# Meng-333/SRADSGAN

Hardware: AMD Instinct MI355X
Metric: training images/sec (216x216, x4) (higher is better)
Workload: dtype f32 (split-bf16 products: 3 bf16 MFMA terms per fp32 multiply, fp32 accumulate)

## Files before the change

### sradsgan_amd/csrc/conv_fast_fprop.hip

```cpp
#include "conv_dev.h"

namespace srhip {

int g_fast_ablate = 0;


template <int BM, int BN, int WM, int WN, int BK, int MATH = 0>
__global__ __launch_bounds__(WM* WN * 64) void fast_conv_kernel(const float* __restrict__ src,
                                                                 const float* __restrict__ wt,
                                                                 const float* __restrict__ bias,
                                                                 const float* __restrict__ residual,
                                                                 const float* __restrict__ rowscale,
                                                                 const float* __restrict__ chanscale,
                                                                 const float* __restrict__ actmask,
                                                                 float* __restrict__ dst, FastGeom g, int nblk_m,
                                                                 int nblk_n) {
  constexpr int NT = WM * WN * 64;
  constexpr int WTM = BM / WM, WTN = BN / WN;
  constexpr int TM = WTM / 32, TN = WTN / 32;
  constexpr int LS = BK + 4;
  constexpr int QPR = BK / 4;
  constexpr int RPP = NT / QPR;
  constexpr int AR = (BM + RPP - 1) / RPP, BR = (BN + RPP - 1) / RPP;
  constexpr int STAGE = (BM + BN) * LS;
// ... 910 lines not shown
    const int orow = pt >> 16, ocol = pt & 0xffff;
    const int arow = orow < pg.PH ? orow * pg.PWP + ocol : 0;
#pragma unroll
    for (int sidx = 0; sidx < 9; ++sidx) {
      const int T = 2 * sidx + wk;
      const int par = T >= 9 ? 1 : 0, tap = T - 9 * par;
      const int th = tap / 3, tw = tap - 3 * th;
      const int a_th = (g.dh0 + th * g.dhs) - pg.lo_h, a_tw = (g.dw0 + tw * g.dws) - pg.lo_w;
      const int pr = arow + a_th * pg.PWP + a_tw;
      aoffS[sidx][t] = par * PATCH_B + pr * 64 + (((2 * khalf) ^ ((pr >> 2) & 3)) << 4);
    }
  }
  int boffk[TN];
#pragma unroll
  for (int u = 0; u < TN; ++u) {
    const int row = u * 32 + l31;
    boffk[u] = 2 * PATCH_B + wk * BSTAGE_B + row * 64 + (((2 * khalf) ^ ((row >> 2) & 3)) << 4);
  }
  f32x16 acc[TM][TN];
#pragma unroll
  for (int t = 0; t < TM; ++t)
#pragma unroll
    for (int u = 0; u < TN; ++u)
#pragma unroll
      for (int r = 0; r < 16; ++r) acc[t][u][r] = 0.f;

  auto do_step = [&](auto sc, auto lastc, int cc0) {
    constexpr int S = decltype(sc)::value;
    constexpr bool LAST = decltype(lastc)::value != 0;
    constexpr int NEWER = S == 0 ? 2 : S == 1 ? 4 : S == 2 ? 3 : (S >= 3 && S <= 5) ? 2 : S == 6 ? (LAST ? 2 : 4) : S == 7 ? (LAST ? 2 : 3) : (LAST ? 0 : 2);
    wait_vmcnt<NEWER>();
    asm volatile("s_waitcnt lgkmcnt(0)" ::: "memory");
    __builtin_amdgcn_s_barrier();
    asm volatile("" ::: "memory");
    if (S == 0) {
      issue_a(1, 0, cc0 + 1);
      issue_a(1, 1, cc0 + 1);
    }
    if (S == 1) issue_a(1, 2, cc0 + 1);
    if (!LAST && S == 5) {
      issue_a(0, 0, cc0 + 2);
      issue_a(0, 1, cc0 + 2);
    }
    if (!LAST && S == 6) issue_a(0, 2, cc0 + 2);
#pragma unroll
    for (int d = 0; d < 2; ++d) {
      constexpr int T0 = 2 * S + 4;
      const int T = T0 + d;
      if (T < 18) issue_b(T % NST, T % 9, cc0 + T / 9);
      else if (!LAST) issue_b(T % NST, (T - 18) % 9, cc0 + 2 + (T - 18) / 9);
    }
    if (S == 2) {
      convert_piece(1, 0);
      convert_piece(1, 1);
    }
    if (S == 3) convert_piece(1, 2);
    if (!LAST && S == 7) {
      convert_piece(0, 0);
      convert_piece(0, 1);
    }
    if (!LAST && S == 8) convert_piece(0, 2);
    const char* sb = lds + ((2 * S) % NST) * BSTAGE_B;
    bf16x8_t ah[TM], al[TM], bh[TN], bl[TN];
#pragma unroll
    for (int t = 0; t < TM; ++t) {
      ah[t] = *reinterpret_cast<const bf16x8_t*>(lds + aoffS[S][t]);
      al[t] = *reinterpret_cast<const bf16x8_t*>(lds + (aoffS[S][t] ^ 16));
    }
#pragma unroll
    for (int u = 0; u < TN; ++u) {
      bh[u] = *reinterpret_cast<const bf16x8_t*>(sb + boffk[u]);
      bl[u] = *reinterpret_cast<const bf16x8_t*>(sb + (boffk[u] ^ 16));
    }
#pragma unroll
    for (int i = 0; i < 3 * TM * TN; ++i) {
      const int grp = i / (TM * TN), t = (i % (TM * TN)) / TN, u = i % TN;
      acc[t][u] = mma16<0>(grp == 0 ? al[t] : ah[t], grp == 1 ? bl[u] : bh[u], acc[t][u]);
    }
  };
  auto do_pair = [&](auto lastc, int cc0) {
    do_step(IC<0>(), lastc, cc0);
    do_step(IC<1>(), lastc, cc0);
    do_step(IC<2>(), lastc, cc0);
    do_step(IC<3>(), lastc, cc0);
    do_step(IC<4>(), lastc, cc0);
    do_step(IC<5>(), lastc, cc0);
    do_step(IC<6>(), lastc, cc0);
    do_step(IC<7>(), lastc, cc0);
    do_step(IC<8>(), lastc, cc0);
  };

  wait_vmcnt<4>();
#pragma unroll
  for (int k = 0; k < MAXP; ++k) convert_piece(0, k);
  for (int cc0 = 0; cc0 + 2 < CC; cc0 += 2) do_pair(IC<0>(), cc0);
  do_pair(IC<1>(), CC - 2);

  __syncthreads();
  {
    float* xl = reinterpret_cast<float*>(lds);
#pragma unroll
    for (int t = 0; t < TM; ++t)
#pragma unroll
      for (int r = 0; r < 16; ++r) xl[((wave * TM + t) * 16 + r) * 64 + lane] = wk ? acc[t][0][r] : acc[t][1][r];
    __syncthreads();
    const int pw = wave ^ 1;
#pragma unroll
    for (int t = 0; t < TM; ++t)
#pragma unroll
      for (int r = 0; r < 16; ++r) {
        const float o = xl[((pw * TM + t) * 16 + r) * 64 + lane];
        acc[t][0][r] = (wk ? acc[t][1][r] : acc[t][0][r]) + o;
      }
    __syncthreads();
  }

  const int flags = EPI >= 0 ? EPI : g.flags;
  constexpr int WTN = 32;
  float* wl = reinterpret_cast<float*>(lds) + wave * (32 * WTN);
  constexpr int QPRW = WTN / 4;
  constexpr int NRD = 32 * QPRW / 64;
#pragma unroll
  for (int t = 0; t < TM; ++t) {
#pragma unroll
    for (int r = 0; r < 16; ++r) wl[((r & 3) + 8 * (r >> 2) + 4 * khalf) * WTN + l31] = acc[t][0][r];
    asm volatile("s_waitcnt lgkmcnt(0)" ::: "memory");
    float4 vq[NRD];
    EpiOps eo[NRD];
    unsigned dpx[NRD];
    int nq[NRD];
    bool okq[NRD];
#pragma unroll
    for (int j = 0; j < NRD; ++j) {
      const int idx = j * 64 + lane;
      const int row = idx / QPRW, cq = idx - row * QPRW;
      vq[j] = *reinterpret_cast<const float4*>(wl + row * WTN + cq * 4);
      const int r = wm * 64 + t * 32 + row;
      const int pt = pix_tab[r];
      const int orow = pt >> 16, ocol = pt & 0xffff;
      const int oh = oh0 + orow, ow = ow0 + ocol;
      const int n = n0 + wk * WTN + cq * 4;
      okq[j] = !(orow >= pg.PH || oh >= g.OH || ow >= g.OW || n >= g.K);
      dpx[j] = okq[j] ? (unsigned)((img * g.Hd + oh) * g.Wd + ow) : 0u;
      nq[j] = okq[j] ? n : 0;
      eo[j] = epi_fetch(dpx[j], nq[j], flags, g, bias, residual, nullptr, actmask, dst, false);
    }
#pragma unroll
    for (int j = 0; j < NRD; ++j)
      if (okq[j]) epi_finish(vq[j], eo[j], dpx[j], nq[j], flags, g, dst, false);
    if (t + 1 < TM) asm volatile("s_waitcnt lgkmcnt(0)" ::: "memory");
  }
}

template <int ND, bool MASK>
__global__ __launch_bounds__(256) void narrow_conv_kernel(const float* __restrict__ src, const float* __restrict__ wt,
                                                           const float* __restrict__ bias, float* __restrict__ dst,
                                                           FastGeom g, int tiles_h, int tiles_w, int lo_h, int lo_w,
                                                           const unsigned long long* __restrict__ smask) {
  constexpr int PW = 16, PH = 16, PWP = PW + 2, PR = (PH + 2) * PWP;
  __shared__ __attribute__((aligned(16))) float4 lds[2][PR * 4];
  const int tid = threadIdx.x;
  const int tpi = tiles_h * tiles_w;
  const int img = blockIdx.x / tpi;
  const int prem = blockIdx.x - img * tpi;
  const int ty = prem / tiles_w, tx = prem - ty * tiles_w;
  const int oh0 = ty * PH, ow0 = tx * PW;
  const int py = tid >> 4, px = tid & 15;

  int soff[6];
  int sdst[6];
  unsigned long long mw[MASK ? 6 : 1];
#pragma unroll
  for (int i = 0; i < 6; ++i) {
    const int e = tid + i * 256;
    soff[i] = -1;
    sdst[i] = 0;
    if (MASK) mw[i] = 0ull;
    if (e < PR * 4) {
      const int row = e >> 2, q = e & 3;
      const int pi = row / PWP, pj = row - pi * PWP;
      const int sh = oh0 + lo_h + pi, sw = ow0 + lo_w + pj;
      sdst[i] = row * 4 + (q ^ (row & 3));
      if (sh >= 0 && sh < g.Hs && sw >= 0 && sw < g.Ws) {
        soff[i] = ((img * g.Hs + sh) * g.Ws + sw) * g.lds + q * 4;
        if (MASK) mw[i] = smask[(img * g.Hs + sh) * g.Ws + sw];
      } else {
        soff[i] = -2;
      }
    }
  }
  const int CC = g.C / 16;
  float4 stage[6];
  auto fetch = [&](int cc) {
#pragma unroll
    for (int i = 0; i < 6; ++i) {
      stage[i] = soff[i] >= 0 ? *reinterpret_cast<const float4*>(src + (size_t)soff[i] + cc * 16) : make_float4(0.f, 0.f, 0.f, 0.f);
      if (MASK) {
        const unsigned b = (unsigned)(mw[i] >> (cc * 16 + (tid & 3) * 4));
        stage[i].x = (b & 1u) ? stage[i].x : stage[i].x * g.slope;
        stage[i].y = (b & 2u) ? stage[i].y : stage[i].y * g.slope;
        stage[i].z = (b & 4u) ? stage[i].z : stage[i].z * g.slope;
        stage[i].w = (b & 8u) ? stage[i].w : stage[i].w * g.slope;
      }
    }
  };
  auto commit = [&](int buf) {
#pragma unroll
    for (int i = 0; i < 6; ++i)
      if (soff[i] != -1) lds[buf][sdst[i]] = stage[i];
  };
  float acc[ND];
#pragma unroll
  for (int n = 0; n < ND; ++n) acc[n] = 0.f;

  fetch(0);
  commit(0);
  __syncthreads();
  for (int cc = 0; cc < CC; ++cc) {
    const int buf = cc & 1;
    if (cc + 1 < CC) fetch(cc + 1);
#pragma unroll 1
    for (int tap = 0; tap < 9; ++tap) {
      {
        const int th = tap / 3, tw = tap - th * 3;
        const int a_th = (g.dh0 + th * g.dhs) - lo_h, a_tw = (g.dw0 + tw * g.dws) - lo_w;
        const int row = (py + a_th) * PWP + px + a_tw;
        const int wk = ((g.kh0 + th * g.khs) * g.KW + (g.kw0 + tw * g.kws)) * g.C + cc * 16;
#pragma unroll
        for (int q = 0; q < 4; ++q) {
          const float4 v = lds[buf][row * 4 + (q ^ (row & 3))];
#pragma unroll
          for (int n = 0; n < ND; ++n) {
            const float* w = wt + (size_t)n * g.ldw + wk + q * 4;
            acc[n] = fmaf(v.x, w[0], acc[n]);
            acc[n] = fmaf(v.y, w[1], acc[n]);
            acc[n] = fmaf(v.z, w[2], acc[n]);
            acc[n] = fmaf(v.w, w[3], acc[n]);
          }
        }
      }
    }
    if (cc + 1 < CC) commit(buf ^ 1);
    __syncthreads();
  }
  const int oh = oh0 + py, ow = ow0 + px;
  if (oh < g.OH && ow < g.OW) {
    const size_t dpix = ((size_t)img * g.Hd + oh) * g.Wd + ow;
#pragma unroll
    for (int n = 0; n < ND; ++n) {
      if (n < g.K) {
        float v = acc[n];
        if (g.flags & SRHIP_EPI_BIAS) v += bias[n];
        if (g.flags & SRHIP_EPI_LRELU) v = v > 0.f ? v : v * g.slope;
        dst[dpix * g.ldd + n] = v;
      }
    }
  }
}

__global__ __launch_bounds__(256) void dot_conv_kernel(const float* __restrict__ src, const float* __restrict__ wt,
                                                        const float* __restrict__ bias, float* __restrict__ dst, FastGeom g) {
  const int lane = threadIdx.x & 63;
  const int m = blockIdx.x * 4 + (threadIdx.x >> 6);
  if (m >= g.M) return;
  const int ow = m % g.OW, t = m / g.OW;
  const int oh = t % g.OH, n = t / g.OH;
  float acc = 0.f;
  for (int th = 0; th < g.TH; ++th) {
    const int sh = oh * g.ss + g.dh0 + th * g.dhs;
    if (sh < 0 || sh >= g.Hs) continue;
    for (int tw = 0; tw < g.TW; ++tw) {
      const int sw = ow * g.ss + g.dw0 + tw * g.dws;
      if (sw < 0 || sw >= g.Ws) continue;
      const float* xp = src + ((size_t)(n * g.Hs + sh) * g.Ws + sw) * g.lds;
      const float* wp = wt + (size_t)((g.kh0 + th * g.khs) * g.KW + (g.kw0 + tw * g.kws)) * g.C;
      for (int c = lane * 4; c < g.C; c += 256) {
        const float4 a = *reinterpret_cast<const float4*>(xp + c);
        const float4 b = *reinterpret_cast<const float4*>(wp + c);
        acc = fmaf(a.x, b.x, acc);
        acc = fmaf(a.y, b.y, acc);
        acc = fmaf(a.z, b.z, acc);
        acc = fmaf(a.w, b.w, acc);
      }
    }
  }
#pragma unroll
  for (int o = 32; o >= 1; o >>= 1) acc += __shfl_xor(acc, o, 64);
  if (lane == 0) {
    float v = acc;
    if (g.flags & SRHIP_EPI_BIAS) v += bias[0];
    if (g.flags & SRHIP_EPI_LRELU) v = v > 0.f ? v : v * g.slope;
    dst[((size_t)(n * g.Hd + oh * g.dsd + g.ph) * g.Wd + ow * g.dsd + g.pw) * g.ldd] = v;
  }
}

__global__ void fast_pack_kernel(const float* __restrict__ w, float* __restrict__ packed, int cout, int cin, int kh,
                                 int kw, int mode) {
  const int idx = blockIdx.x * blockDim.x + threadIdx.x;
  const int total = cout * cin * kh * kw;
  if (idx >= total) return;
  const int khkw = kh * kw;
  if (mode == 0) {
    const int co = idx / (khkw * cin);
    const int rem = idx - co * khkw * cin;
    const int tap = rem / cin, ci = rem - tap * cin;
    fast_pack_store(packed, total, idx, w[((size_t)co * cin + ci) * khkw + tap], cout, cin, khkw);
  } else {
    const int ci = idx / (khkw * cout);
    const int rem = idx - ci * khkw * cout;
    const int tap = rem / cout, co = rem - tap * cout;
    fast_pack_store(packed, total, idx, w[((size_t)co * cin + ci) * khkw + tap], cin, cout, khkw);
  }
}

static bool shape_ok(int csrc, int kh, int kw) { return csrc % 16 == 0 && kh * kw <= 32 && kh == kw; }
bool fast_fwd_ok(int cin, int cout, int kh, int kw) { return shape_ok(cin, kh, kw); }
bool fast_dgrad_ok(int cin, int cout, int kh, int kw) { return shape_ok(cout, kh, kw); }
bool fast_wgrad_ok(int cin, int cout, int kh, int kw) { return cin % 16 == 0 && cout % 4 == 0 && kh == kw; }

int fast_pack_weight(const float* w, float* packed, int cout, int cin, int kh, int kw, int mode, hipStream_t st) {
  const long total = (long)cout * cin * kh * kw;
  hipLaunchKernelGGL(fast_pack_kernel, dim3(cdiv(total, 256)), dim3(256), 0, st, w, packed, cout, cin, kh, kw, mode);
  return check_launch("fast_pack_weight");
}

thread_local Dst2Request g_dst2_req;
thread_local ResRequest g_res_req;
thread_local PhaseRequest g_phase_req;
thread_local SrcMaskRequest g_src_mask_req;
int g_conv_math = 0;
int g_patch_ks = 1;
int g_fast_cfg = 0;
int g_phase_batch = 1;

static bool plan_patch(const FastGeom& g, PatchGeom* pg, double min_eff = 0.70) {
  if (g.TH != 3 || g.TW != 3 || g.ss != 1 || g.dsd != 1 || g.ph != 0 || g.pw != 0) return false;
  if ((g.dhs != 1 && g.dhs != -1) || (g.dws != 1 && g.dws != -1)) return false;
  if (g.Hd != g.OH || g.Wd != g.OW) return false;
  double best = 0.0;
  for (int pw = 4; pw <= 64 && pw <= g.OW + 3; ++pw) {
    int ph = 128 / pw;
    if (ph > g.OH) ph = g.OH;
    if (ph < 1 || (ph + 2) * (pw + 2) > 192) continue;
    const long tiles = (long)cdiv(g.OH, ph) * cdiv(g.OW, pw);
    const double eff = (double)g.OH * g.OW / ((double)tiles * 128.0) + 1e-6 * (double)(pw - pw % 16) / pw;
    if (eff > best + 1e-9) {
      best = eff;
      pg->PH = ph; pg->PW = pw;
    }
  }
  if (best < min_eff || best <= 0.0) return false;
  pg->tiles_h = cdiv(g.OH, pg->PH);
  pg->tiles_w = cdiv(g.OW, pg->PW);
  pg->PWP = pg->PW + 2;
  pg->PR = (pg->PH + 2) * pg->PWP;
  pg->npieces = cdiv(pg->PR, 16);
  pg->lo_h = g.dhs > 0 ? g.dh0 : g.dh0 + 2 * g.dhs;
  pg->lo_w = g.dws > 0 ? g.dw0 : g.dw0 + 2 * g.dws;
  const int a = pg->PW >> 4;
  const int nfull = pg->PH * a < 8 ? pg->PH * a : 8;
  auto base = [&](int q) { return ((q / a) * pg->PWP + (q % a) * 16) & 15; };
  int fin[8], nf = 0, singles[8], ns = 0;
  bool used[8] = {false, false, false, false, false, false, false, false};
  for (int q = 0; q < nfull; ++q) {
    if (used[q]) continue;
    used[q] = true;
    int partner = -1;
    for (int p2 = q + 1; p2 < nfull; ++p2)
      if (!used[p2] && base(p2) == base(q)) {
        partner = p2;
        break;
      }
    if (partner >= 0) {
      used[partner] = true;
      fin[nf++] = q;
      fin[nf++] = partner;
    } else {
      singles[ns++] = q;
    }
  }
  for (int i = 0; i < ns; ++i) fin[nf++] = singles[i];
  for (int q = nfull; q < 8; ++q) fin[nf++] = q;
  pg->gmap = 0;
  for (int i = 0; i < 8; ++i) pg->gmap |= (unsigned)(fin[i] & 15) << (4 * i);
  return true;
}

long pp_sign_tiles(int n, int h, int w, int cout) {
  if (cout < 128 || cout % 128 != 0) return 0;
  FastGeom g;
// ... 409 lines not shown
```

### sradsgan_amd/csrc/conv_igemm.hip

```cpp
#include "common.h"
#include "conv_internal.h"

namespace srhip {
int g_headconv_rows = 4;
}
namespace srhip {

constexpr int BK = 16;

struct ConvGeom {
  int N, H, W, C;
  int Ho, Wo, K;
  int KH, KW;
  int so, pad, dv;
  int ldx, ldy, ldr, ldw;
  int Ktot;
  int M;
  float slope;
  int flags;
  int accumulate;
};

__device__ inline f32x16 mfma32(float a, float b, f32x16 c) {
  return __builtin_amdgcn_mfma_f32_32x32x2f32(a, b, c, 0, 0, 0);
// ... 487 lines not shown
          const float* tq = tile + px0 * HEAD_TLD + 4 * cq;
          const float4 o0 = *reinterpret_cast<const float4*>(tq), o1 = *reinterpret_cast<const float4*>(tq + 8 * HEAD_TLD);
          const float4 o2 = *reinterpret_cast<const float4*>(tq + 16 * HEAD_TLD), o3 = *reinterpret_cast<const float4*>(tq + 24 * HEAD_TLD);
          __builtin_amdgcn_fence(__ATOMIC_SEQ_CST, "wavefront");
          __builtin_amdgcn_wave_barrier();
          float* yq = yg + (unsigned)(px0 * ldy + 4 * cq);
          if (ow0 + px0 < W) *reinterpret_cast<float4*>(yq) = o0;
          if (ow0 + px0 + 8 < W) *reinterpret_cast<float4*>(yq + (unsigned)(8 * ldy)) = o1;
          if (ow0 + px0 + 16 < W) *reinterpret_cast<float4*>(yq + (unsigned)(16 * ldy)) = o2;
          if (ow0 + px0 + 24 < W) *reinterpret_cast<float4*>(yq + (unsigned)(24 * ldy)) = o3;
        } else {
#pragma unroll 2
          for (int t = 0; t < 16; ++t) {
            const int px = 2 * t + half;
            const float o = tile[px * HEAD_TLD + l31];
            if (ow0 + px < W && co0 + 32 * hh + l31 < cout) yg[(unsigned)(px * ldy + l31)] = o;
          }
          __builtin_amdgcn_fence(__ATOMIC_SEQ_CST, "wavefront");
          __builtin_amdgcn_wave_barrier();
        }
      }
      if (MASK == 1 && lane < 32 && ow0 + lane < W)
        rec[(size_t)r * W + ow0 + lane] = ((unsigned long long)wrec[1] << 32) | wrec[0];
    }
  }
}

template <int MASK>
static void launch_headconv(dim3 grid, size_t lds, hipStream_t st, int cin, const float* x, const float* packed, const float* bias, float* y,
                            unsigned long long* rec, int n, int h, int w, int cout, int ldx, int ldy, int ldw, float slope, int flags,
                            int rows_per_block, int rows_chunk) {
  auto kernel = cin == 1 ? headconv_fwd_kernel<MASK, 1> : (cin == 2 ? headconv_fwd_kernel<MASK, 2> : headconv_fwd_kernel<MASK, 3>);
  hipLaunchKernelGGL(kernel, grid, dim3(256), lds, st, x, packed, bias, y, rec, n, h, w, cout, ldx, ldy, ldw, slope, flags, rows_per_block,
                     rows_chunk);
}

template <bool BITS>
__global__ __launch_bounds__(256) void wgrad_smallcin_kernel(const float* __restrict__ x, const float* __restrict__ dy,
                                                              const float* __restrict__ ymask,
                                                              const unsigned long long* __restrict__ ybits, float slope,
                                                              float* __restrict__ partial, float* __restrict__ bias_partial,
                                                              int N, int H, int W, int cin,
                                                              int cout, int ldx, int ldy, int rows_per_split) {
  extern __shared__ float xs[];
  const int tid = threadIdx.x, lane = tid & 63;
  const int wave = __builtin_amdgcn_readfirstlane(tid >> 6);
  const int l31 = lane & 31, half = lane >> 5;
  const int co0 = blockIdx.y * 64;
  const int ktot = 9 * cin;
  const int rowlen = (W + 2) * cin;
  int koff = -1;
  if (l31 < ktot) {
    const int tap = l31 / cin, ci = l31 - tap * cin;
    const int kh = tap / 3, kw = tap - kh * 3;
    koff = kh * rowlen + kw * cin + ci;
  }
  const bool c0ok = co0 + l31 < cout, c1ok = co0 + 32 + l31 < cout;
  f32x16 acc0, acc1;
#pragma unroll
  for (int r = 0; r < 16; ++r) acc0[r] = acc1[r] = 0.f;
  float bs0 = 0.f, bs1 = 0.f;
  const int r_begin = blockIdx.x * rows_per_split, r_end = min(r_begin + rows_per_split, N * H);
  for (int r = r_begin; r < r_end; ++r) {
    const int n = r / H, oh = r - n * H;
    __syncthreads();
    for (int e0 = tid; e0 < 3 * rowlen; e0 += 256 * 8) {
      float v[8];
#pragma unroll
      for (int u = 0; u < 8; ++u) {
        const int e = e0 + 256 * u;
        const int kh = e / rowlen, rem = e - kh * rowlen;
        const int col = rem / cin, ci = rem - col * cin;
        const int ih = oh + kh - 1, iw = col - 1;
        v[u] = (e < 3 * rowlen && ih >= 0 && ih < H && iw >= 0 && iw < W) ? x[((size_t)(n * H + ih) * W + iw) * ldx + ci] : 0.f;
      }
#pragma unroll
      for (int u = 0; u < 8; ++u)
        if (e0 + 256 * u < 3 * rowlen) xs[e0 + 256 * u] = v[u];
    }
    __syncthreads();
    const float* drow = dy + (size_t)r * W * ldy + co0 + l31;
    const float* yrow = (!BITS && ymask) ? ymask + (size_t)r * W * ldy + co0 + l31 : nullptr;
    const unsigned long long* brow = BITS ? ybits + (size_t)r * W : nullptr;
    constexpr int PF = 4;
    for (int owb = 2 * wave; owb < W; owb += 8 * PF) {
      float d0[PF], d1[PF], y0[PF], y1[PF];
      unsigned long long m[PF];
#pragma unroll
      for (int u = 0; u < PF; ++u) {
        const int p = owb + 8 * u + half;
        const bool pok = p < W;
        d0[u] = (pok && c0ok) ? drow[(size_t)p * ldy] : 0.f;
        d1[u] = (pok && c1ok) ? drow[(size_t)p * ldy + 32] : 0.f;
        m[u] = ~0ull;
        y0[u] = y1[u] = 1.f;
        if (BITS) {
          if (pok) m[u] = brow[p];
        } else if (yrow != nullptr) {
          if (pok && c0ok) y0[u] = yrow[(size_t)p * ldy];
          if (pok && c1ok) y1[u] = yrow[(size_t)p * ldy + 32];
        }
      }
#pragma unroll
      for (int u = 0; u < PF; ++u) {
        if (owb + 8 * u < W) {
          const int p = owb + 8 * u + half;
          const bool pok = p < W;
          float e0 = d0[u], e1 = d1[u];
          if (BITS) {
            if (!((m[u] >> l31) & 1ull)) e0 *= slope;
            if (!((m[u] >> (32 + l31)) & 1ull)) e1 *= slope;
          } else if (yrow != nullptr) {
            if (!(y0[u] > 0.f)) e0 *= slope;
            if (!(y1[u] > 0.f)) e1 *= slope;
          }
          const float b = (pok && koff >= 0) ? xs[p * cin + koff] : 0.f;
          bs0 += e0;
          bs1 += e1;
          acc0 = __builtin_amdgcn_mfma_f32_32x32x2f32(e0, b, acc0, 0, 0, 0);
          acc1 = __builtin_amdgcn_mfma_f32_32x32x2f32(e1, b, acc1, 0, 0, 0);
        }
      }
    }
  }
  __syncthreads();
  float* red = xs;
#pragma unroll
  for (int r = 0; r < 16; ++r) {
    const int row = (r & 3) + 8 * (r >> 2) + 4 * half;
    red[(wave * 64 + row) * 32 + l31] = acc0[r];
    red[(wave * 64 + 32 + row) * 32 + l31] = acc1[r];
  }
  __syncthreads();
  for (int e = tid; e < 64 * 32; e += 256) {
    const int co = e >> 5, k = e & 31;
    if (k < ktot && co0 + co < cout)
      partial[((size_t)blockIdx.x * cout + co0 + co) * ktot + k] =
          (red[e] + red[2048 + e]) + (red[4096 + e] + red[6144 + e]);
  }
  if (bias_partial != nullptr) {
    __syncthreads();
    red[(wave * 2 + half) * 64 + l31] = bs0;
    red[(wave * 2 + half) * 64 + 32 + l31] = bs1;
    __syncthreads();
    if (tid < 64 && co0 + tid < cout) {
      float s = 0.f;
#pragma unroll
      for (int j = 0; j < 8; ++j) s += red[j * 64 + tid];
      bias_partial[(size_t)blockIdx.x * cout + co0 + tid] = s;
    }
  }
}

template <int ND>
__global__ __launch_bounds__(576) void wgrad_narrow_kernel(const float* __restrict__ x, const float* __restrict__ dy,
                                                            float* __restrict__ partial, int N, int H, int W, int cin,
                                                            int ldx, int ldy, int tiles_h, int tiles_w) {
  constexpr int PW = 16, PH = 16, PWP = PW + 2, NPX = (PH + 2) * PWP;
  constexpr int NLD = (NPX * 16 + 575) / 576;
  typedef float f32x2 __attribute__((ext_vector_type(2)));
  extern __shared__ float xs[];
  float4* dys = reinterpret_cast<float4*>(xs + NPX * 64);
  const int tid = threadIdx.x;
  const int rg = tid / 192, kh = (tid - rg * 192) >> 6, ci = tid & 63;
  const int row0 = rg == 0 ? 0 : (rg == 1 ? 6 : 11), row1 = rg == 0 ? 6 : (rg == 1 ? 11 : 16);
  const int ci0 = blockIdx.y * 64;
  const int npatch = N * tiles_h * tiles_w;
  const int tpi = tiles_h * tiles_w;
  f32x2 acc01[3], acc23[3];
#pragma unroll
  for (int k = 0; k < 3; ++k) acc01[k] = acc23[k] = f32x2{0.f, 0.f};
  float4 stage[NLD];
  float4 dstage = make_float4(0.f, 0.f, 0.f, 0.f);
  auto fetch = [&](int pid) {
    const int n = pid / tpi, prem = pid - n * tpi;
    const int ty = prem / tiles_w, tx = prem - ty * tiles_w;
#pragma unroll
    for (int i = 0; i < NLD; ++i) {
      const int e = tid + i * 576;
      const int px = e >> 4, q = e & 15;
      const int pi = px / PWP, pj = px - pi * PWP;
      const int ih = ty * PH - 1 + pi, iw = tx * PW - 1 + pj;
      stage[i] = make_float4(0.f, 0.f, 0.f, 0.f);
      if (e < NPX * 16 && ih >= 0 && ih < H && iw >= 0 && iw < W)
        stage[i] = *reinterpret_cast<const float4*>(x + ((size_t)(n * H + ih) * W + iw) * ldx + ci0 + q * 4);
    }
    dstage = make_float4(0.f, 0.f, 0.f, 0.f);
    if (tid < PH * PW) {
      const int oh = ty * PH + (tid >> 4), ow = tx * PW + (tid & 15);
      if (oh < H && ow < W) {
        const float* dp = dy + ((size_t)(n * H + oh) * W + ow) * ldy;
        dstage.x = dp[0];
        if (ND > 1) dstage.y = dp[1];
        if (ND > 2) dstage.z = dp[2];
        if (ND > 3) dstage.w = dp[3];
      }
    }
  };
  int pid = blockIdx.x;
  if (pid < npatch) fetch(pid);
  for (; pid < npatch; pid += gridDim.x) {
    __syncthreads();
#pragma unroll
    for (int i = 0; i < NLD; ++i) {
      const int e = tid + i * 576;
      if (e < NPX * 16) *reinterpret_cast<float4*>(xs + (e >> 4) * 64 + (e & 15) * 4) = stage[i];
    }
    if (tid < PH * PW) dys[tid] = dstage;
    __syncthreads();
    if (pid + (int)gridDim.x < npatch) fetch(pid + gridDim.x);
    for (int py = row0; py < row1; ++py) {
      const float* xr = xs + ((py + kh) * PWP) * 64 + ci;
      float xv[PWP];
#pragma unroll
      for (int j = 0; j < PWP; ++j) xv[j] = xr[j * 64];
#pragma unroll
      for (int px = 0; px < PW; ++px) {
        const float4 d = dys[py * PW + px];
        const f32x2 d01 = {d.x, d.y}, d23 = {d.z, d.w};
#pragma unroll
        for (int kw = 0; kw < 3; ++kw) {
          const f32x2 vv = {xv[px + kw], xv[px + kw]};
          acc01[kw] = __builtin_elementwise_fma(vv, d01, acc01[kw]);
          if (ND > 2) acc23[kw] = __builtin_elementwise_fma(vv, d23, acc23[kw]);
        }
      }
    }
  }
  __syncthreads();
  float* red = xs;
#pragma unroll
  for (int kw = 0; kw < 3; ++kw) {
    const int tap = kh * 3 + kw;
    red[((rg * 4 + 0) * 9 + tap) * 64 + ci] = acc01[kw].x;
    if (ND > 1) red[((rg * 4 + 1) * 9 + tap) * 64 + ci] = acc01[kw].y;
    if (ND > 2) red[((rg * 4 + 2) * 9 + tap) * 64 + ci] = acc23[kw].x;
    if (ND > 3) red[((rg * 4 + 3) * 9 + tap) * 64 + ci] = acc23[kw].y;
  }
  __syncthreads();
  const int ktot = 9 * cin;
  for (int e = tid; e < ND * 9 * 64; e += 576) {
    const int c = e & 63, tap = (e >> 6) % 9, co = e / (9 * 64);
    const int o = (co * 9 + tap) * 64 + c;
    const float v = (red[o] + red[4 * 9 * 64 + o]) + red[2 * 4 * 9 * 64 + o];
    partial[(size_t)blockIdx.x * ND * ktot + (size_t)co * ktot + tap * cin + ci0 + c] = v;
  }
}

__global__ __launch_bounds__(256) void wgrad_reduce_kernel(const float* __restrict__ partial, float* __restrict__ dw,
                                                            int nsplit, int cout, int cin, int khkw, int ktot) {
  __shared__ float red[256];
  const int o = threadIdx.x & 15, sub = threadIdx.x >> 4;
  const int idx = blockIdx.x * 16 + o;
  const int total = cout * ktot;
  float s0 = 0.f, s1 = 0.f;
  if (idx < total) {
    int i = sub;
    for (; i + 16 < nsplit; i += 32) {
      s0 += partial[(size_t)i * total + idx];
      s1 += partial[(size_t)(i + 16) * total + idx];
    }
    for (; i < nsplit; i += 16) s0 += partial[(size_t)i * total + idx];
  }
  red[threadIdx.x] = s0 + s1;
  __syncthreads();
  if (sub == 0 && idx < total) {
    float s = 0.f;
#pragma unroll
    for (int j = 0; j < 16; ++j) s += red[j * 16 + o];
    const int co = idx / ktot, kcol = idx - co * ktot;
    const int tap = kcol / cin, ci = kcol - tap * cin;
    dw[((size_t)co * cin + ci) * khkw + tap] = s;
  }
}

__global__ void pack_weight_kernel(const float* __restrict__ w, float* __restrict__ packed, int cout, int cin,
                                   int kh, int kw, int mode, int ld) {
  int idx = blockIdx.x * blockDim.x + threadIdx.x;
  int csrc = mode == 0 ? cin : cout;
  int cdst = mode == 0 ? cout : cin;
  int rows = kh * kw * csrc;
  if (idx >= rows * ld) return;
  int row = idx / ld, col = idx - row * ld;
  float v = 0.f;
  if (col < cdst) {
    int tap = row / csrc, cs = row - tap * csrc;
    int a = tap / kw, b = tap - a * kw;
    if (mode == 0)
      v = w[(((size_t)col * cin + cs) * kh + a) * kw + b];
    else
      v = w[(((size_t)cs * cin + col) * kh + (kh - 1 - a)) * kw + (kw - 1 - b)];
  }
  packed[idx] = v;
}

template <int BM, int BN, int WM, int WN>
static int launch_fprop(const float* src, const float* wt, const float* bias, const float* residual,
                        const float* rowscale, float* dst, const ConvGeom& g, bool vec, hipStream_t st) {
  int blocks = cdiv(g.M, BM) * cdiv(g.K, BN);
  if (vec)
    hipLaunchKernelGGL((igemm_fprop_kernel<BM, BN, WM, WN, true>), dim3(blocks), dim3(256), 0, st, src, wt, bias,
                       residual, rowscale, dst, g);
  else
    hipLaunchKernelGGL((igemm_fprop_kernel<BM, BN, WM, WN, false>), dim3(blocks), dim3(256), 0, st, src, wt, bias,
                       residual, rowscale, dst, g);
  return check_launch("igemm_fprop");
}

static int run_fprop(const float* src, const float* wt, const float* bias, const float* residual,
                     const float* rowscale, float* dst, const ConvGeom& g, hipStream_t st) {
  const bool vec = (g.C % 4 == 0) && (g.ldx % 4 == 0);
  if (g.M <= 0) return SRHIP_OK;
  if (g.K <= 32) return launch_fprop<128, 32, 4, 1>(src, wt, bias, residual, rowscale, dst, g, vec, st);
  long blocks128 = (long)cdiv(g.M, 128) * cdiv(g.K, 128);
  if (g.K >= 128 && blocks128 >= 512) return launch_fprop<128, 128, 2, 2>(src, wt, bias, residual, rowscale, dst, g, vec, st);
  long blocks64n = (long)cdiv(g.M, 128) * cdiv(g.K, 64);
  if (blocks64n >= 512) return launch_fprop<128, 64, 2, 2>(src, wt, bias, residual, rowscale, dst, g, vec, st);
  return launch_fprop<64, 64, 2, 2>(src, wt, bias, residual, rowscale, dst, g, vec, st);
}

template <int BM, int BN, int WM, int WN>
static int launch_wgrad(const float* x, const float* dy, float* partial, const ConvGeom& g, int nsplit, int cps,
                        bool va, bool vb, hipStream_t st) {
  int blocks = cdiv(g.K, BM) * cdiv(g.Ktot, BN) * nsplit;
#define SRHIP_WG(VA_, VB_)                                                                                     \
  hipLaunchKernelGGL((igemm_wgrad_kernel<BM, BN, WM, WN, VA_, VB_>), dim3(blocks), dim3(256), 0, st, x, dy, \
                     partial, g, nsplit, cps)
  if (va && vb)
    SRHIP_WG(true, true);
  else if (va)
    SRHIP_WG(true, false);
  else if (vb)
    SRHIP_WG(false, true);
  else
    SRHIP_WG(false, false);
#undef SRHIP_WG
  return check_launch("igemm_wgrad");
}

struct WgradPlan {
  int bm, bn, nsplit, chunks_per_split;
};

static WgradPlan plan_wgrad(int M, int cout, int ktot) {
  WgradPlan p;
  p.bm = cout > 64 ? 128 : (cout > 32 ? 64 : 32);
  p.bn = p.bm == 32 ? 128 : 64;
  long tiles = (long)cdiv(cout, p.bm) * cdiv(ktot, p.bn);
  int nchunks = cdiv(M, BK);
  long want = (1024 + tiles - 1) / tiles;
  if (cout <= 4 && want < 256) want = 256;
  long maxsplit = (nchunks + 15) / 16;
  long ns = want < 1 ? 1 : want;
  if (ns > maxsplit) ns = maxsplit;
  if (ns < 1) ns = 1;
  p.chunks_per_split = (int)((nchunks + ns - 1) / ns);
  p.nsplit = cdiv(nchunks, p.chunks_per_split);
  return p;
}

}

namespace srhip {

int legacy_packed_ld(int cdst) { return ((cdst + 31) / 32) * 32; }

int legacy_pack_weight(const float* w, float* packed, int cout, int cin, int kh, int kw, int mode, void* stream) {
  SRHIP_REQUIRE(w && packed && cout > 0 && cin > 0 && kh > 0 && kw > 0 && (mode == 0 || mode == 1),
                "pack_weight: bad argument");
  int csrc = mode == 0 ? cin : cout, cdst = mode == 0 ? cout : cin;
  int ld = legacy_packed_ld(cdst);
  long total = (long)kh * kw * csrc * ld;
  hipLaunchKernelGGL(pack_weight_kernel, dim3(cdiv(total, 256)), dim3(256), 0, as_stream(stream), w, packed, cout,
                     cin, kh, kw, mode, ld);
  return check_launch("pack_weight");
}

int legacy_conv2d_fwd(const float* x, const float* packed, const float* bias, const float* residual,
                     const float* rowscale, float* y, int n, int h, int w, int cin, int cout, int kh, int kw,
                     int stride, int pad, int ldx, int ldy, int ldr, float slope, int flags, void* stream) {
  SRHIP_REQUIRE(x && packed && y, "conv2d_fwd: null tensor");
  SRHIP_REQUIRE(n >= 0 && h > 0 && w > 0 && cin > 0 && cout > 0 && kh > 0 && kw > 0 && stride > 0 && pad >= 0,
                "conv2d_fwd: bad geometry");
  SRHIP_REQUIRE(ldx >= cin && ldy >= cout, "conv2d_fwd: row stride smaller than channel count");
  SRHIP_REQUIRE(!(flags & SRHIP_EPI_BIAS) || bias, "conv2d_fwd: EPI_BIAS without bias");
  SRHIP_REQUIRE(!(flags & SRHIP_EPI_RESIDUAL) || (residual && ldr >= cout), "conv2d_fwd: EPI_RESIDUAL without residual");
  SRHIP_REQUIRE(!(flags & SRHIP_EPI_ROWSCALE) || rowscale, "conv2d_fwd: EPI_ROWSCALE without rowscale");
  ConvGeom g;
  g.N = n; g.H = h; g.W = w; g.C = cin;
  g.Ho = (h + 2 * pad - kh) / stride + 1;
  g.Wo = (w + 2 * pad - kw) / stride + 1;
  SRHIP_REQUIRE(g.Ho > 0 && g.Wo > 0, "conv2d_fwd: empty output");
  g.K = cout; g.KH = kh; g.KW = kw; g.so = stride; g.pad = pad; g.dv = 1;
  g.ldx = ldx; g.ldy = ldy; g.ldr = ldr; g.ldw = legacy_packed_ld(cout);
  g.Ktot = kh * kw * cin;
  long M = (long)n * g.Ho * g.Wo;
  SRHIP_REQUIRE(M < (1L << 31) && (long)n * h * w < (1L << 31), "conv2d_fwd: pixel count overflows int32");
  g.M = (int)M; g.slope = slope; g.flags = flags; g.accumulate = 0;
  if (head_conv_shape(n, h, w, cin, kh, kw, stride, pad) && !(flags & ~(SRHIP_EPI_BIAS | SRHIP_EPI_LRELU))) {
    const int rpb = g_headconv_rows > 0 ? g_headconv_rows : 1;
    size_t lds = 0;
    const int rchunk = headconv_rows_chunk(w, cin, rpb, &lds);
    launch_headconv<0>(dim3(cdiv((long)n * h, rpb), cdiv(cout, 64)), lds, as_stream(stream), cin, x, packed, bias, y, nullptr, n, h, w, cout, ldx,
                       ldy, g.ldw, slope, flags, rpb, rchunk);
    return check_launch("headconv_fwd");
  }
  return run_fprop(x, packed, bias, residual, rowscale, y, g, as_stream(stream));
}

bool head_conv_shape(int n, int h, int w, int cin, int kh, int kw, int stride, int pad) {
  return n > 0 && h > 0 && w > 0 && cin > 0 && cin <= 3 && kh == 3 && kw == 3 && stride == 1 && pad == 1 && (long)n * h * w >= 65536 &&
         (long)n * h * w < (1L << 31) && (size_t)3 * (w + 2) * cin * sizeof(float) <= 32 * 1024;
}

int legacy_headconv_fwd_mask(const float* x, const float* packed, const float* bias, float* y, void* rec_out, const void* rec_in, int n,
                             int h, int w, int cin, int cout, int ldx, int ldy, float slope, int flags, void* stream) {
  SRHIP_REQUIRE(x && packed && y && ((rec_out != nullptr) != (rec_in != nullptr)), "conv2d_fwd_head_mask: null tensor / exactly one of mask_out, mask_in");
  SRHIP_REQUIRE(head_conv_shape(n, h, w, cin, 3, 3, 1, 1) && cout == 64 && ldx >= cin && ldy >= cout,
                "conv2d_fwd_head_mask: shape not served (srhip_conv2d_head_mask_ok)");
  SRHIP_REQUIRE(rec_out ? (flags == (SRHIP_EPI_BIAS | SRHIP_EPI_LRELU) && bias != nullptr) : flags == 0,
                "conv2d_fwd_head_mask: mask_out goes with bias + LeakyReLU, mask_in with a plain epilogue");
  const int rpb = g_headconv_rows > 0 ? g_headconv_rows : 1;
  const dim3 grid(cdiv((long)n * h, rpb), 1);
  size_t lds = 0;
  const int rchunk = headconv_rows_chunk(w, cin, rpb, &lds);
  const int ldw = legacy_packed_ld(cout);
  if (rec_out)
    launch_headconv<1>(grid, lds, as_stream(stream), cin, x, packed, bias, y, static_cast<unsigned long long*>(rec_out), n, h, w, cout, ldx, ldy, ldw,
                       slope, flags, rpb, rchunk);
  else
    launch_headconv<2>(grid, lds, as_stream(stream), cin, x, packed, bias, y, static_cast<unsigned long long*>(const_cast<void*>(rec_in)), n, h, w,
                       cout, ldx, ldy, ldw, slope, flags, rpb, rchunk);
  return check_launch("headconv_fwd_mask");
}

int legacy_conv2d_dgrad(const float* dy, const float* packed, float* dx, int n, int h, int w, int cin, int cout,
                       int kh, int kw, int stride, int pad, int ldy, int ldx, int accumulate, void* stream) {
  SRHIP_REQUIRE(dy && packed && dx, "conv2d_dgrad: null tensor");
  SRHIP_REQUIRE(n >= 0 && h > 0 && w > 0 && cin > 0 && cout > 0 && kh > 0 && kw > 0 && stride > 0 && pad >= 0,
                "conv2d_dgrad: bad geometry");
  SRHIP_REQUIRE(pad <= kh - 1 && pad <= kw - 1, "conv2d_dgrad: pad > kernel-1 unsupported");
  SRHIP_REQUIRE(ldy >= cout && ldx >= cin, "conv2d_dgrad: row stride smaller than channel count");
  ConvGeom g;
  g.N = n;
  g.H = (h + 2 * pad - kh) / stride + 1;
  g.W = (w + 2 * pad - kw) / stride + 1;
  SRHIP_REQUIRE(g.H > 0 && g.W > 0, "conv2d_dgrad: empty dy");
  g.C = cout; g.Ho = h; g.Wo = w; g.K = cin; g.KH = kh; g.KW = kw;
  g.so = 1; g.pad = kh - 1 - pad; g.dv = stride;
  SRHIP_REQUIRE(kh == kw, "conv2d_dgrad: square kernels only");
  g.ldx = ldy; g.ldy = ldx; g.ldr = 0; g.ldw = legacy_packed_ld(cin);
  g.Ktot = kh * kw * cout;
  long M = (long)n * h * w;
  SRHIP_REQUIRE(M < (1L << 31), "conv2d_dgrad: pixel count overflows int32");
  g.M = (int)M; g.slope = 0.f; g.flags = 0; g.accumulate = accumulate ? 1 : 0;
  return run_fprop(dy, packed, nullptr, nullptr, nullptr, dx, g, as_stream(stream));
}

size_t legacy_conv2d_wgrad_workspace(int n, int h, int w, int cin, int cout, int kh, int kw, int stride, int pad) {
  int ho = (h + 2 * pad - kh) / stride + 1, wo = (w + 2 * pad - kw) / stride + 1;
  long M = (long)n * ho * wo;
  if (M <= 0) return 0;
  WgradPlan p = plan_wgrad((int)M, cout, kh * kw * cin);
  return (size_t)p.nsplit * cout * kh * kw * cin * sizeof(float);
}

size_t legacy_conv2d_wgrad_bias_workspace(int n, int h, int w, int cin, int cout, int kh, int kw, int stride, int pad) {
  const int ho = (h + 2 * pad - kh) / stride + 1, wo = (w + 2 * pad - kw) / stride + 1;
  const long M = (long)n * ho * wo;
  if (M <= 0) return 0;
  return (size_t)plan_wgrad((int)M, cout, kh * kw * cin).nsplit * cout * sizeof(float);
}

int legacy_conv2d_wgrad(const float* x, const float* dy, float* dw, void* workspace, size_t workspace_bytes, int n,
                       int h, int w, int cin, int cout, int kh, int kw, int stride, int pad, int ldx, int ldy,
                       void* stream, float* db, float* bias_ws, int* bias_done, const float* ymask, float slope, const void* ybits) {
  if (bias_done) *bias_done = 0;
  SRHIP_REQUIRE(!ymask || (db && bias_ws && bias_done && cin <= 3 && kh == 3 && kw == 3 && stride == 1 && pad == 1 &&
                           (long)n * h * w >= 65536 && (size_t)3 * (w + 2) * cin * sizeof(float) <= 32 * 1024),
                "conv2d_wgrad: the fused activation mask is built for the 3-channel 3x3 head convs at full image size (with bias)");
  SRHIP_REQUIRE(!ybits || (!ymask && cout == 64 && head_conv_shape(n, h, w, cin, kh, kw, stride, pad)),
                "conv2d_wgrad: the activation record is built for the 3-channel 3x3 head convs to 64 channels at full image size");
  SRHIP_REQUIRE(x && dy && dw, "conv2d_wgrad: null tensor");
  SRHIP_REQUIRE(n > 0 && h > 0 && w > 0 && cin > 0 && cout > 0 && kh > 0 && kw > 0 && stride > 0 && pad >= 0,
                "conv2d_wgrad: bad geometry");
  SRHIP_REQUIRE(ldx >= cin && ldy >= cout, "conv2d_wgrad: row stride smaller than channel count");
  ConvGeom g;
  g.N = n; g.H = h; g.W = w; g.C = cin;
  g.Ho = (h + 2 * pad - kh) / stride + 1;
  g.Wo = (w + 2 * pad - kw) / stride + 1;
  SRHIP_REQUIRE(g.Ho > 0 && g.Wo > 0, "conv2d_wgrad: empty output");
  g.K = cout; g.KH = kh; g.KW = kw; g.so = stride; g.pad = pad; g.dv = 1;
  g.ldx = ldx; g.ldy = ldy; g.ldr = 0; g.ldw = 0; g.Ktot = kh * kw * cin;
  long M = (long)n * g.Ho * g.Wo;
  SRHIP_REQUIRE(M < (1L << 31) && (long)n * h * w < (1L << 31), "conv2d_wgrad: pixel count overflows int32");
  g.M = (int)M; g.slope = 0.f; g.flags = 0; g.accumulate = 0;
  WgradPlan p = plan_wgrad(g.M, cout, g.Ktot);
  size_t need = (size_t)p.nsplit * cout * g.Ktot * sizeof(float);
  if (!workspace || workspace_bytes < need) {
    set_error("conv2d_wgrad: workspace %zu bytes < required %zu", workspace_bytes, need);
    return SRHIP_ERR_WORKSPACE;
  }
  float* partial = static_cast<float*>(workspace);
  hipStream_t st = as_stream(stream);
  if (cin <= 3 && kh == 3 && kw == 3 && stride == 1 && pad == 1 && g.M >= 65536 &&
      (size_t)3 * (w + 2) * cin * sizeof(float) <= 32 * 1024) {
    const int rows = n * h;
    int ns = p.nsplit < rows ? p.nsplit : rows;
    const int rps = cdiv(rows, ns);
    ns = cdiv(rows, rps);
    const bool fuse_bias = db != nullptr && bias_ws != nullptr && bias_done != nullptr;
    if (ybits)
      hipLaunchKernelGGL(wgrad_smallcin_kernel<true>, dim3(ns, 1), dim3(256), (size_t)32 * 1024, st, x, dy, (const float*)nullptr,
                         static_cast<const unsigned long long*>(ybits), slope, partial, fuse_bias ? bias_ws : nullptr, n, h, w, cin, cout, ldx,
                         ldy, rps);
    else
      hipLaunchKernelGGL(wgrad_smallcin_kernel<false>, dim3(ns, cdiv(cout, 64)), dim3(256), (size_t)32 * 1024, st, x, dy, ymask,
                         (const unsigned long long*)nullptr, slope, partial, fuse_bias ? bias_ws : nullptr, n, h, w, cin, cout, ldx, ldy, rps);
    int rc0 = check_launch("wgrad_smallcin");
    if (rc0) return rc0;
    long total0 = (long)cout * g.Ktot;
    hipLaunchKernelGGL(wgrad_reduce_kernel, dim3(cdiv(total0, 16)), dim3(256), 0, st, partial, dw, ns, cout, cin, kh * kw,
                       g.Ktot);
    if (fuse_bias) {
      hipLaunchKernelGGL(wgrad_reduce_kernel, dim3(cdiv(cout, 16)), dim3(256), 0, st, bias_ws, db, ns, cout, 1, 1, 1);
      *bias_done = 1;
    }
    return check_launch("wgrad_reduce");
  }
  if (cout <= 4 && cin % 64 == 0 && ldx % 4 == 0 && ((uintptr_t)x & 15) == 0 && kh == 3 && kw == 3 && stride == 1 && pad == 1 &&
      g.M >= 65536 && p.nsplit >= 64) {
    const int th = cdiv(h, 16), tw = cdiv(w, 16);
    const int ns = p.nsplit < 256 ? p.nsplit : 256;
    const size_t lds_bytes = (size_t)(18 * 18 * 64 + 256 * 4) * sizeof(float);
#define SRHIP_WN(ND_)                                                                                                    \
  do {                                                                                                                   \
    static bool attr_set = false;                                                                                        \
    if (!attr_set) {                                                                                                     \
      (void)hipFuncSetAttribute(reinterpret_cast<const void*>(wgrad_narrow_kernel<ND_>),                                 \
                                hipFuncAttributeMaxDynamicSharedMemorySize, (int)lds_bytes);                             \
      attr_set = true;                                                                                                   \
    }                                                                                                                    \
    hipLaunchKernelGGL(wgrad_narrow_kernel<ND_>, dim3(ns, cin / 64), dim3(576), lds_bytes, st, x, dy, partial, n, h, w,  \
                       cin, ldx, ldy, th, tw);                                                                           \
  } while (0)
    if (cout == 1) SRHIP_WN(1);
    else if (cout == 2) SRHIP_WN(2);
    else if (cout == 3) SRHIP_WN(3);
    else SRHIP_WN(4);
#undef SRHIP_WN
    int rc1 = check_launch("wgrad_narrow");
    if (rc1) return rc1;
    hipLaunchKernelGGL(wgrad_reduce_kernel, dim3(cdiv((long)cout * g.Ktot, 16)), dim3(256), 0, st, partial, dw, ns, cout, cin,
                       kh * kw, g.Ktot);
    return check_launch("wgrad_reduce");
  }
  const bool va = (cout % 4 == 0) && (ldy % 4 == 0);
  const bool vb = (cin % 4 == 0) && (ldx % 4 == 0);
  int rc;
  if (p.bm == 128)
    rc = launch_wgrad<128, 64, 2, 2>(x, dy, partial, g, p.nsplit, p.chunks_per_split, va, vb, st);
  else if (p.bm == 64)
    rc = launch_wgrad<64, 64, 2, 2>(x, dy, partial, g, p.nsplit, p.chunks_per_split, va, vb, st);
  else
    rc = launch_wgrad<32, 128, 1, 4>(x, dy, partial, g, p.nsplit, p.chunks_per_split, va, vb, st);
  if (rc) return rc;
  long total = (long)cout * g.Ktot;
  hipLaunchKernelGGL(wgrad_reduce_kernel, dim3(cdiv(total, 16)), dim3(256), 0, st, partial, dw, p.nsplit, cout, cin,
                     kh * kw, g.Ktot);
  return check_launch("wgrad_reduce");
}

}
```

Baseline: 695.3.

## Retune narrow conv kernels: SGPR weight FMAs, new thread mapping, smaller wgrad tiles, headconv dgrad

The narrow forward conv now remaps threads to pixels in a different interleaved pattern and changes the LDS swizzle. Its FMAs are forced through inline asm so the weights come from scalar registers. The narrow wgrad kernel uses 8-row tiles with 384 threads, a waves-per-eu hint, scalar FMAs, and a higher split count with a two-way reduction. Separately, dgrad for head-conv shapes now goes through the headconv kernel instead of generic fprop. These changes target LDS bank conflicts, register pressure and occupancy, but mix several unrelated ideas, and the inline asm limits what the compiler can schedule.

```diff
diff --git a/sradsgan_amd/csrc/conv_fast_fprop.hip b/sradsgan_amd/csrc/conv_fast_fprop.hip
--- a/sradsgan_amd/csrc/conv_fast_fprop.hip
+++ b/sradsgan_amd/csrc/conv_fast_fprop.hip
@@ -1086,6 +1086,8 @@
   }
 }
 
+__device__ __forceinline__ void fmac_sgpr(float& acc, float v, float w) { asm("v_fmac_f32 %0, %2, %1" : "+v"(acc) : "v"(v), "s"(w)); }
+
 template <int ND, bool MASK>
 __global__ __launch_bounds__(256) void narrow_conv_kernel(const float* __restrict__ src, const float* __restrict__ wt,
                                                            const float* __restrict__ bias, float* __restrict__ dst,
@@ -1099,7 +1101,10 @@
   const int prem = blockIdx.x - img * tpi;
   const int ty = prem / tiles_w, tx = prem - ty * tiles_w;
   const int oh0 = ty * PH, ow0 = tx * PW;
-  const int py = tid >> 4, px = tid & 15;
+  const int l5 = tid & 31;
+  const int odd_group = (l5 >= 4 && l5 < 12) || (l5 >= 16 && l5 < 20) || l5 >= 28;
+  const int py = (tid >> 5) * 2 + odd_group;
+  const int px = l5 < 4 ? l5 : l5 < 12 ? l5 - 4 : l5 < 20 ? l5 - 8 : l5 < 28 ? l5 - 12 : l5 - 16;
 
   int soff[6];
   int sdst[6];
@@ -1114,7 +1119,7 @@
       const int row = e >> 2, q = e & 3;
       const int pi = row / PWP, pj = row - pi * PWP;
       const int sh = oh0 + lo_h + pi, sw = ow0 + lo_w + pj;
-      sdst[i] = row * 4 + (q ^ (row & 3));
+      sdst[i] = row * 4 + (q ^ ((row >> 2) & 3));
       if (sh >= 0 && sh < g.Hs && sw >= 0 && sw < g.Ws) {
         soff[i] = ((img * g.Hs + sh) * g.Ws + sw) * g.lds + q * 4;
         if (MASK) mw[i] = smask[(img * g.Hs + sh) * g.Ws + sw];
@@ -1162,14 +1167,14 @@
         const int wk = ((g.kh0 + th * g.khs) * g.KW + (g.kw0 + tw * g.kws)) * g.C + cc * 16;
 #pragma unroll
         for (int q = 0; q < 4; ++q) {
-          const float4 v = lds[buf][row * 4 + (q ^ (row & 3))];
+          const float4 v = lds[buf][row * 4 + (q ^ ((row >> 2) & 3))];
 #pragma unroll
           for (int n = 0; n < ND; ++n) {
             const float* w = wt + (size_t)n * g.ldw + wk + q * 4;
-            acc[n] = fmaf(v.x, w[0], acc[n]);
-            acc[n] = fmaf(v.y, w[1], acc[n]);
-            acc[n] = fmaf(v.z, w[2], acc[n]);
-            acc[n] = fmaf(v.w, w[3], acc[n]);
+            fmac_sgpr(acc[n], v.x, w[0]);
+            fmac_sgpr(acc[n], v.y, w[1]);
+            fmac_sgpr(acc[n], v.z, w[2]);
+            fmac_sgpr(acc[n], v.w, w[3]);
           }
         }
       }
diff --git a/sradsgan_amd/csrc/conv_igemm.hip b/sradsgan_amd/csrc/conv_igemm.hip
--- a/sradsgan_amd/csrc/conv_igemm.hip
+++ b/sradsgan_amd/csrc/conv_igemm.hip
@@ -663,24 +663,29 @@
   }
 }
 
+__device__ __forceinline__ void fmac_vgpr(float& acc, float a, float b) { asm("v_fmac_f32 %0, %1, %2" : "+v"(acc) : "v"(a), "v"(b)); }
+constexpr int WN_PW = 16, WN_PH = 8, WN_PWP = WN_PW + 2, WN_NPX = (WN_PH + 2) * WN_PWP;
+constexpr int WN_THREADS = 2 * 3 * 64;
+constexpr size_t WN_LDS_BYTES = (size_t)(WN_NPX * 64 + WN_PH * WN_PW * 4) * sizeof(float);
 template <int ND>
-__global__ __launch_bounds__(576) void wgrad_narrow_kernel(const float* __restrict__ x, const float* __restrict__ dy,
-                                                            float* __restrict__ partial, int N, int H, int W, int cin,
-                                                            int ldx, int ldy, int tiles_h, int tiles_w) {
-  constexpr int PW = 16, PH = 16, PWP = PW + 2, NPX = (PH + 2) * PWP;
-  constexpr int NLD = (NPX * 16 + 575) / 576;
-  typedef float f32x2 __attribute__((ext_vector_type(2)));
+__global__ __launch_bounds__(WN_THREADS) __attribute__((amdgpu_waves_per_eu(3))) void wgrad_narrow_kernel(
+    const float* __restrict__ x, const float* __restrict__ dy, float* __restrict__ partial, int N, int H, int W, int cin, int ldx, int ldy,
+    int tiles_h, int tiles_w) {
+  constexpr int PW = WN_PW, PH = WN_PH, PWP = WN_PWP, NPX = WN_NPX;
+  constexpr int NLD = (NPX * 16 + WN_THREADS - 1) / WN_THREADS;
   extern __shared__ float xs[];
   float4* dys = reinterpret_cast<float4*>(xs + NPX * 64);
   const int tid = threadIdx.x;
   const int rg = tid / 192, kh = (tid - rg * 192) >> 6, ci = tid & 63;
-  const int row0 = rg == 0 ? 0 : (rg == 1 ? 6 : 11), row1 = rg == 0 ? 6 : (rg == 1 ? 11 : 16);
+  const int row0 = rg * (PH / 2), row1 = row0 + PH / 2;
   const int ci0 = blockIdx.y * 64;
   const int npatch = N * tiles_h * tiles_w;
   const int tpi = tiles_h * tiles_w;
-  f32x2 acc01[3], acc23[3];
-#pragma unroll
-  for (int k = 0; k < 3; ++k) acc01[k] = acc23[k] = f32x2{0.f, 0.f};
+  float acc[3][ND];
+#pragma unroll
+  for (int k = 0; k < 3; ++k)
+#pragma unroll
+    for (int c = 0; c < ND; ++c) acc[k][c] = 0.f;
   float4 stage[NLD];
   float4 dstage = make_float4(0.f, 0.f, 0.f, 0.f);
   auto fetch = [&](int pid) {
@@ -688,7 +693,7 @@
     const int ty = prem / tiles_w, tx = prem - ty * tiles_w;
 #pragma unroll
     for (int i = 0; i < NLD; ++i) {
-      const int e = tid + i * 576;
+      const int e = tid + i * WN_THREADS;
       const int px = e >> 4, q = e & 15;
       const int pi = px / PWP, pj = px - pi * PWP;
       const int ih = ty * PH - 1 + pi, iw = tx * PW - 1 + pj;
@@ -714,7 +719,7 @@
     __syncthreads();
 #pragma unroll
     for (int i = 0; i < NLD; ++i) {
-      const int e = tid + i * 576;
+      const int e = tid + i * WN_THREADS;
       if (e < NPX * 16) *reinterpret_cast<float4*>(xs + (e >> 4) * 64 + (e & 15) * 4) = stage[i];
     }
     if (tid < PH * PW) dys[tid] = dstage;
@@ -723,18 +728,18 @@
     for (int py = row0; py < row1; ++py) {
       const float* xr = xs + ((py + kh) * PWP) * 64 + ci;
       float xv[PWP];
+      float4 d[PW];
+#pragma unroll
+      for (int px = 0; px < PW; ++px) d[px] = dys[py * PW + px];
 #pragma unroll
       for (int j = 0; j < PWP; ++j) xv[j] = xr[j * 64];
 #pragma unroll
       for (int px = 0; px < PW; ++px) {
-        const float4 d = dys[py * PW + px];
-        const f32x2 d01 = {d.x, d.y}, d23 = {d.z, d.w};
-#pragma unroll
-        for (int kw = 0; kw < 3; ++kw) {
-          const f32x2 vv = {xv[px + kw], xv[px + kw]};
-          acc01[kw] = __builtin_elementwise_fma(vv, d01, acc01[kw]);
-          if (ND > 2) acc23[kw] = __builtin_elementwise_fma(vv, d23, acc23[kw]);
-        }
+        const float dc[4] = {d[px].x, d[px].y, d[px].z, d[px].w};
+#pragma unroll
+        for (int kw = 0; kw < 3; ++kw)
+#pragma unroll
+          for (int c = 0; c < ND; ++c) fmac_vgpr(acc[kw][c], xv[px + kw], dc[c]);
       }
     }
   }
@@ -743,17 +748,15 @@
 #pragma unroll
   for (int kw = 0; kw < 3; ++kw) {
     const int tap = kh * 3 + kw;
-    red[((rg * 4 + 0) * 9 + tap) * 64 + ci] = acc01[kw].x;
-    if (ND > 1) red[((rg * 4 + 1) * 9 + tap) * 64 + ci] = acc01[kw].y;
-    if (ND > 2) red[((rg * 4 + 2) * 9 + tap) * 64 + ci] = acc23[kw].x;
-    if (ND > 3) red[((rg * 4 + 3) * 9 + tap) * 64 + ci] = acc23[kw].y;
+#pragma unroll
+    for (int c = 0; c < ND; ++c) red[((rg * 4 + c) * 9 + tap) * 64 + ci] = acc[kw][c];
   }
   __syncthreads();
   const int ktot = 9 * cin;
-  for (int e = tid; e < ND * 9 * 64; e += 576) {
+  for (int e = tid; e < ND * 9 * 64; e += WN_THREADS) {
     const int c = e & 63, tap = (e >> 6) % 9, co = e / (9 * 64);
     const int o = (co * 9 + tap) * 64 + c;
-    const float v = (red[o] + red[4 * 9 * 64 + o]) + red[2 * 4 * 9 * 64 + o];
+    const float v = red[o] + red[4 * 9 * 64 + o];
     partial[(size_t)blockIdx.x * ND * ktot + (size_t)co * ktot + tap * cin + ci0 + c] = v;
   }
 }
@@ -860,7 +863,7 @@
   long tiles = (long)cdiv(cout, p.bm) * cdiv(ktot, p.bn);
   int nchunks = cdiv(M, BK);
   long want = (1024 + tiles - 1) / tiles;
-  if (cout <= 4 && want < 256) want = 256;
+  if (cout <= 4 && want < 512) want = 512;
   long maxsplit = (nchunks + 15) / 16;
   long ns = want < 1 ? 1 : want;
   if (ns > maxsplit) ns = maxsplit;
@@ -965,6 +968,14 @@
   long M = (long)n * h * w;
   SRHIP_REQUIRE(M < (1L << 31), "conv2d_dgrad: pixel count overflows int32");
   g.M = (int)M; g.slope = 0.f; g.flags = 0; g.accumulate = accumulate ? 1 : 0;
+  if (!accumulate && head_conv_shape(n, h, w, cout, kh, kw, stride, pad)) {
+    const int rpb = g_headconv_rows > 0 ? g_headconv_rows : 1;
+    size_t lds = 0;
+    const int rchunk = headconv_rows_chunk(w, cout, rpb, &lds);
+    launch_headconv<0>(dim3(cdiv((long)n * h, rpb), cdiv(cin, 64)), lds, as_stream(stream), cout, dy, packed, nullptr, dx, nullptr, n, h, w, cin,
+                       ldy, ldx, g.ldw, 0.f, 0, rpb, rchunk);
+    return check_launch("headconv_dgrad");
+  }
   return run_fprop(dy, packed, nullptr, nullptr, nullptr, dx, g, as_stream(stream));
 }
 
@@ -1041,20 +1052,11 @@
   }
   if (cout <= 4 && cin % 64 == 0 && ldx % 4 == 0 && ((uintptr_t)x & 15) == 0 && kh == 3 && kw == 3 && stride == 1 && pad == 1 &&
       g.M >= 65536 && p.nsplit >= 64) {
-    const int th = cdiv(h, 16), tw = cdiv(w, 16);
-    const int ns = p.nsplit < 256 ? p.nsplit : 256;
-    const size_t lds_bytes = (size_t)(18 * 18 * 64 + 256 * 4) * sizeof(float);
-#define SRHIP_WN(ND_)                                                                                                    \
-  do {                                                                                                                   \
-    static bool attr_set = false;                                                                                        \
-    if (!attr_set) {                                                                                                     \
-      (void)hipFuncSetAttribute(reinterpret_cast<const void*>(wgrad_narrow_kernel<ND_>),                                 \
-                                hipFuncAttributeMaxDynamicSharedMemorySize, (int)lds_bytes);                             \
-      attr_set = true;                                                                                                   \
-    }                                                                                                                    \
-    hipLaunchKernelGGL(wgrad_narrow_kernel<ND_>, dim3(ns, cin / 64), dim3(576), lds_bytes, st, x, dy, partial, n, h, w,  \
-                       cin, ldx, ldy, th, tw);                                                                           \
-  } while (0)
+    const int th = cdiv(h, WN_PH), tw = cdiv(w, WN_PW);
+    const int ns = p.nsplit < 512 ? p.nsplit : 512;
+#define SRHIP_WN(ND_)                                                                                                        \
+  hipLaunchKernelGGL(wgrad_narrow_kernel<ND_>, dim3(ns, cin / 64), dim3(WN_THREADS), WN_LDS_BYTES, st, x, dy, partial, n, h, w, cin, ldx, \
+                     ldy, th, tw)
     if (cout == 1) SRHIP_WN(1);
     else if (cout == 2) SRHIP_WN(2);
     else if (cout == 3) SRHIP_WN(3);
```

New measurement: 699.1, median of 6. About the same (+0.5%).
